# yatpor/bpc_baseline

Hardware: NVIDIA B200
Metric: matched+triangulated scenes/s with the ROI crops of every match (crops/s alongside) (higher is better)
Workload: dtype f64 geometry / u8+f32 crops

## Files before the change

### bpc_baseline_b200/_lib.py

```python
from __future__ import annotations

import ctypes as C
import os

HERE = os.path.dirname(os.path.abspath(__file__))
LIB_PATH = os.environ.get('BPC_LIB') or os.path.join(HERE, 'libbpc_b200.so')

_p = C.c_void_p
_i = C.c_int
_f = C.c_float
_sz = C.c_size_t

SIGNATURES = {
    'bpc_abi_version': (_i, []),
    'bpc_error_string': (C.c_char_p, [_i]),
    'bpc_launch_count': (C.c_ulonglong, []),
    'bpc_fundamental': (_i, [_p, _p, _i, _p, _p]),
    'bpc_cost_tensor': (_i, [_p, _p, _p, _i, _i, _p, _p]),
    'bpc_match_objects': (_i, [_p, _i, _i, _i, _i, _f, _p, _p, _p]),
    'bpc_match_workspace_bytes': (_sz, [_i, _i]),
    'bpc_match_triangulate': (_i, [_p, _p, _p, _p, _i, _i, _f, _i, C.c_double, _p, _p, _p, _p, _p, _p, _p, _sz, _p]),
    'bpc_pack_records_bytes': (_sz, [_i, _i]),
    'bpc_pack_records': (_i, [_p, _p, _p, _p, _p, _p, _i, _i, _i, _p, _p]),
    'bpc_triangulate': (_i, [_p, _p, _i, _p, _p]),
    'bpc_projection': (_i, [_p, _p, _i, _p, _p]),
    'bpc_reprojection_error': (_i, [_p, _p, _p, _i, _p, _p]),
    'bpc_epipolar_error': (_i, [_p, _p, _p, _i, _p, _p]),
    'bpc_epipolar_error_full': (_i, [_p, _p, _i, _p, _p]),
    'bpc_triangulate_views': (_i, [_p, _p, _i, _i, _p, _p]),
    'bpc_box_centers': (_i, [_p, _i, _p, _p]),
    'bpc_detections_from_yolo': (_i, [_p, _p, _p, _p, _i, _i, _f, _i, _p, _p, _p, _p]),
    'bpc_build_rois': (_i, [_p, _p, _p, _p, _i, _i, _i, _p, _p, _p]),
    'bpc_train_rois': (_i, [_p, _p, _p, _p, _i, _i, _i, _p, _p]),
    'bpc_roi_crop_workspace_bytes': (_sz, [_i, _i]),
    'bpc_roi_crop': (_i, [_p, _i, _i, _i, _p, _i, _p, _i, _i, _p, _i, _p, _p, _p, _p, _sz, _p]),
    'bpc_roi_crop_u8': (_i, [_p, _i, _i, _i, _p, _i, _p, _i, _i, _p, _p, _p, _p, _sz, _p]),
    'bpc_roi_crop_bf16': (_i, [_p, _i, _i, _i, _p, _i, _p, _i, _i, _p, _i, _p, _p, _p, _p, _sz, _p]),
    'bpc_normalise_lut': (_i, [_p, _p, _p, _p]),
    'bpc_crops_normalise': (_i, [_p, _p, _i, _i, _i, _p, _p, _p]),
    'bpc_color_jitter': (_i, [_p, _i, _i, _p, _p, _i, _p, _p, _p]),
}

_lib = None
ABI_VERSION = 2


class BpcError(RuntimeError):
    pass


def load():
    global _lib
    if _lib is not None:
        return _lib
    if not os.path.exists(LIB_PATH):
        raise BpcError(f'{LIB_PATH} not found: build it with `python -m bpc_baseline_b200.build` '
                       '(or __graft_entry__.build()); there is no CPU fallback')
    lib = C.CDLL(LIB_PATH)
    for name, (res, args) in SIGNATURES.items():
        fn = getattr(lib, name)
        fn.restype = res
        fn.argtypes = args
    if lib.bpc_abi_version() != ABI_VERSION:
        raise BpcError(f'ABI version mismatch: library {lib.bpc_abi_version()}, binding {ABI_VERSION}')
    _lib = lib
    return lib


def check(code: int, what: str):
    if code != 0:
        msg = load().bpc_error_string(code).decode()
        raise BpcError(f'{what} failed with code {code}: {msg}')


def launch_count() -> int:
    return int(load().bpc_launch_count())
```

### bpc_baseline_b200/batched.py

```python
from __future__ import annotations

import ctypes as C
from dataclasses import dataclass
from typing import Optional, Sequence

import numpy as np
import torch

from . import _lib

MEAN = (0.485, 0.456, 0.406)
STD = (0.229, 0.224, 0.225)


def _chk(t: torch.Tensor, dtype, name: str, ndim: Optional[int] = None):
    if not isinstance(t, torch.Tensor):
        raise TypeError(f'{name}: expected a torch.Tensor, got {type(t).__name__}')
    if not t.is_cuda:
        raise RuntimeError(f'{name}: must be a CUDA tensor (no CPU fallback)')
    if t.dtype != dtype:
        raise RuntimeError(f'{name}: dtype {t.dtype}, expected {dtype}')
    if not t.is_contiguous():
        raise RuntimeError(f'{name}: must be contiguous')
    if ndim is not None and t.dim() != ndim:
# ... 212 lines not shown
    e = torch.empty((n,), dtype=torch.float64, device=F.device)
    with torch.cuda.device(F.device):
        _lib.check(_lib.load().bpc_epipolar_error(_p(F), _p(pt1), _p(pt2), n, _p(e), _stream(F.device)), 'bpc_epipolar_error')
    return e


def epipolar_error_full(F: torch.Tensor, pts: torch.Tensor) -> torch.Tensor:
    _chk(F, torch.float64, 'F', 4); _chk(pts, torch.float64, 'pts', 3)
    n = F.shape[0]
    if tuple(F.shape) != (n, 3, 3, 3) or tuple(pts.shape) != (n, 3, 2):
        raise RuntimeError('expected F [n,3,3,3] and pts [n,3,2]')
    e = torch.empty((n,), dtype=torch.float64, device=F.device)
    with torch.cuda.device(F.device):
        _lib.check(_lib.load().bpc_epipolar_error_full(_p(F), _p(pts), n, _p(e), _stream(F.device)), 'bpc_epipolar_error_full')
    return e


def triangulate_views(P: torch.Tensor, pts: torch.Tensor) -> torch.Tensor:
    _chk(P, torch.float64, 'P', 4); _chk(pts, torch.float64, 'pts', 3)
    n, V = P.shape[0], P.shape[1]
    if tuple(P.shape) != (n, V, 3, 4) or tuple(pts.shape) != (n, V, 2) or not 2 <= V <= 8:
        raise RuntimeError('expected P [n,V,3,4] and pts [n,V,2] with 2 <= V <= 8')
    X = torch.empty((n, 3), dtype=torch.float64, device=P.device)
    with torch.cuda.device(P.device):
        _lib.check(_lib.load().bpc_triangulate_views(_p(P), _p(pts), n, V, _p(X), _stream(P.device)), 'bpc_triangulate_views')
    return X


def build_rois(boxes: torch.Tensor, idx: torch.Tensor, n: torch.Tensor, image_of_scene: torch.Tensor,
               rois: Optional[torch.Tensor] = None) -> tuple[torch.Tensor, torch.Tensor]:
    _chk(boxes, torch.int32, 'boxes', 4); _chk(idx, torch.int32, 'idx', 3); _chk(n, torch.int32, 'n', 1)
    _chk(image_of_scene, torch.int32, 'image_of_scene', 2)
    S, _, D, _ = boxes.shape
    K = idx.shape[1]
    dev = boxes.device
    if rois is None:
        rois = torch.empty((S * K * 3, 5), dtype=torch.int32, device=dev)
    else:
        _chk(rois, torch.int32, 'rois', 2)
        if rois.shape[0] < S * K * 3 or rois.shape[1] != 5:
            raise RuntimeError('rois must be int32 [>= S*Kmax*3, 5]')
    offs = torch.empty((S + 1,), dtype=torch.int32, device=dev)
    with torch.cuda.device(dev):
        _lib.check(_lib.load().bpc_build_rois(_p(boxes), _p(idx), _p(n), _p(image_of_scene), S, D, K, _p(offs), _p(rois),
                                              _stream(dev)), 'bpc_build_rois')
    return rois, offs


_LUT_CACHE: dict = {}


def normalise_lut(device, mean: Sequence[float] = MEAN, std: Sequence[float] = STD) -> torch.Tensor:
    device = torch.device(device)
    key = (device.index if device.index is not None else torch.cuda.current_device(), tuple(mean), tuple(std))
    if key not in _LUT_CACHE:
        lut = torch.empty((3, 256), dtype=torch.float32, device=device)
        m = (C.c_float * 3)(*[float(np.float32(v)) for v in mean])
        s = (C.c_float * 3)(*[float(np.float32(v)) for v in std])
        with torch.cuda.device(device):
            _lib.check(_lib.load().bpc_normalise_lut(m, s, _p(lut), _stream(device)), 'bpc_normalise_lut')
        _LUT_CACHE[key] = lut
    return _LUT_CACHE[key]


_WS_CACHE: dict = {}
MAX_ROIS_PER_LAUNCH = 32768
MAX_TARGET = 1024
MAX_ROI_WIDTH = 8192


def _crop_workspace(dev, R: int, T: int) -> torch.Tensor:
    need = int(_lib.load().bpc_roi_crop_workspace_bytes(int(R), int(T)))
    key = (dev.index if dev.index is not None else torch.cuda.current_device(), int(torch.cuda.current_stream(dev).cuda_stream))
    ws = _WS_CACHE.get(key)
    if ws is None or ws.numel() < need:
        ws = torch.empty((max(need, 1 << 16),), dtype=torch.uint8, device=dev)
        _WS_CACHE[key] = ws
    return ws


def _chk_status(status, R: int) -> None:
    if status is not None:
        _chk(status, torch.int32, 'status', 1)
        if status.shape[0] < R:
            raise RuntimeError('status must hold one int32 per ROI')


def _crop_args(images, rois, T, fill):
    _chk(images, torch.uint8, 'images', 4); _chk(rois, torch.int32, 'rois', 2)
    B, H, W, ch = images.shape
    if ch != 3 or rois.shape[1] != 5:
        raise RuntimeError('images must be [B,H,W,3] and rois [R,5]')
    if not 1 <= int(T) <= MAX_TARGET:
        raise RuntimeError(f'target size must be in 1..{MAX_TARGET}')
    f = (C.c_uint8 * 3)(*[int(v) for v in fill])
    return B, H, W, rois.shape[0], f


def roi_crop(images: torch.Tensor, rois: torch.Tensor, T: int = 256, fill=(255, 255, 255), swap_rb: bool = True,
             lut: Optional[torch.Tensor] = None, n_rois: Optional[torch.Tensor] = None, roi_first: int = 0,
             out: Optional[torch.Tensor] = None, status: Optional[torch.Tensor] = None) -> torch.Tensor:
    B, H, W, R, f = _crop_args(images, rois, T, fill)
    dev = images.device
    if lut is None:
        lut = normalise_lut(dev)
    _chk_lut(lut, dev)
    if out is None:
        out = torch.empty((R, 3, T, T), dtype=torch.float32, device=dev)
    else:
        _chk(out, torch.float32, 'out', 4)
        if out.shape[0] < R or tuple(out.shape[1:]) != (3, T, T):
            raise RuntimeError('out must be [>=R,3,T,T]')
        _chk_device(out, dev, 'out')
    _chk_status(status, R)
    if n_rois is not None:
        _chk(n_rois, torch.int32, 'n_rois')
    ws = _crop_workspace(dev, min(R, MAX_ROIS_PER_LAUNCH), T)
    with torch.cuda.device(dev):
        for lo in range(0, R, MAX_ROIS_PER_LAUNCH):
            r = min(MAX_ROIS_PER_LAUNCH, R - lo)
            _lib.check(_lib.load().bpc_roi_crop(_p(images), B, H, W, _p(rois[lo:lo + r]), r, _p(n_rois), int(roi_first) + lo, int(T),
                                                f, int(bool(swap_rb)), _p(lut), _p(out[lo:lo + r]),
                                                _p(status[lo:lo + r]) if status is not None else None,
                                                _p(ws), ws.numel(), _stream(dev)), 'bpc_roi_crop')
    return out


def roi_crop_bf16(images: torch.Tensor, rois: torch.Tensor, T: int = 256, fill=(255, 255, 255), swap_rb: bool = True,
                  lut: Optional[torch.Tensor] = None, n_rois: Optional[torch.Tensor] = None, roi_first: int = 0,
                  out: Optional[torch.Tensor] = None, status: Optional[torch.Tensor] = None) -> torch.Tensor:
    B, H, W, R, f = _crop_args(images, rois, T, fill)
    dev = images.device
    if lut is None:
        lut = normalise_lut(dev)
    _chk_lut(lut, dev)
    if out is None:
        out = torch.empty((R, 3, T, T), dtype=torch.bfloat16, device=dev, memory_format=torch.channels_last)
    else:
        if out.dtype != torch.bfloat16 or not out.is_cuda or out.dim() != 4 or out.shape[0] < R or tuple(out.shape[1:]) != (3, T, T) \
                or not out.is_contiguous(memory_format=torch.channels_last):
            raise RuntimeError('out must be a channels_last bfloat16 CUDA tensor [>=R,3,T,T]')
        _chk_device(out, dev, 'out')
    _chk_status(status, R)
    if n_rois is not None:
        _chk(n_rois, torch.int32, 'n_rois')
    ws = _crop_workspace(dev, min(R, MAX_ROIS_PER_LAUNCH), T)
    with torch.cuda.device(dev):
        for lo in range(0, R, MAX_ROIS_PER_LAUNCH):
            r = min(MAX_ROIS_PER_LAUNCH, R - lo)
            _lib.check(_lib.load().bpc_roi_crop_bf16(_p(images), B, H, W, _p(rois[lo:lo + r]), r, _p(n_rois), int(roi_first) + lo, int(T),
                                                     f, int(bool(swap_rb)), _p(lut), out[lo:lo + r].data_ptr(),
                                                     _p(status[lo:lo + r]) if status is not None else None,
                                                     _p(ws), ws.numel(), _stream(dev)), 'bpc_roi_crop_bf16')
    return out


def roi_crop_u8(images: torch.Tensor, rois: torch.Tensor, T: int = 256, fill=(255, 255, 255),
                   n_rois: Optional[torch.Tensor] = None, roi_first: int = 0, out: Optional[torch.Tensor] = None,
                status: Optional[torch.Tensor] = None) -> torch.Tensor:
    B, H, W, R, f = _crop_args(images, rois, T, fill)
    dev = images.device
    if out is None:
        out = torch.empty((R, T, T, 3), dtype=torch.uint8, device=dev)
    else:
        _chk(out, torch.uint8, 'out', 4)
        if out.shape[0] < R or tuple(out.shape[1:]) != (T, T, 3):
            raise RuntimeError('out must be uint8 [>=R,T,T,3]')
        _chk_device(out, dev, 'out')
    _chk_status(status, R)
    if n_rois is not None:
        _chk(n_rois, torch.int32, 'n_rois')
    ws = _crop_workspace(dev, min(R, MAX_ROIS_PER_LAUNCH), T)
    with torch.cuda.device(dev):
        for lo in range(0, R, MAX_ROIS_PER_LAUNCH):
            r = min(MAX_ROIS_PER_LAUNCH, R - lo)
            _lib.check(_lib.load().bpc_roi_crop_u8(_p(images), B, H, W, _p(rois[lo:lo + r]), r, _p(n_rois), int(roi_first) + lo, int(T),
                                                   f, _p(out[lo:lo + r]), _p(status[lo:lo + r]) if status is not None else None,
                                                   _p(ws), ws.numel(), _stream(dev)), 'bpc_roi_crop_u8')
    return out


def crops_normalise(sources: Sequence[torch.Tensor], T: int, swap_rb: bool = True, lut: Optional[torch.Tensor] = None,
                    out: Optional[torch.Tensor] = None, device=None) -> torch.Tensor:
    if not 1 <= len(sources) <= 16:
        raise RuntimeError('1..16 sources')
    for s in sources:
        _chk(s, torch.uint8, 'sources[*]', 4)
        if tuple(s.shape[1:]) != (T, T, 3):
            raise RuntimeError('every source must be uint8 [n,T,T,3]')
    dev = torch.device(device) if device is not None else sources[0].device
    if dev.type == 'cuda' and dev.index is None:
        dev = torch.device('cuda', torch.cuda.current_device())
    if lut is None:
        lut = normalise_lut(dev)
    _chk_lut(lut, dev)
    total = sum(int(s.shape[0]) for s in sources)
    if out is None:
        out = torch.empty((total, 3, T, T), dtype=torch.float32, device=dev)
    else:
        _chk(out, torch.float32, 'out', 4)
        if out.shape[0] < total or tuple(out.shape[1:]) != (3, T, T):
            raise RuntimeError('out must be [>=sum(n_s),3,T,T]')
        _chk_device(out, dev, 'out')
    ptrs = (C.c_void_p * len(sources))(*[s.data_ptr() if s.shape[0] else None for s in sources])
    counts = (C.c_int32 * len(sources))(*[int(s.shape[0]) for s in sources])
    with torch.cuda.device(dev):
        _lib.check(_lib.load().bpc_crops_normalise(ptrs, counts, len(sources), int(T), int(bool(swap_rb)), _p(lut), _p(out),
                                                   _stream(dev)), 'bpc_crops_normalise')
    return out


def color_jitter(canvases: torch.Tensor, order: torch.Tensor, factors: torch.Tensor, swap_rb: bool = False,
                 lut: Optional[torch.Tensor] = None, out: Optional[torch.Tensor] = None) -> torch.Tensor:
    _chk(canvases, torch.uint8, 'canvases', 4); _chk(order, torch.int32, 'order', 2); _chk(factors, torch.float32, 'factors', 2)
    n, T = canvases.shape[0], canvases.shape[1]
    if tuple(canvases.shape[1:]) != (T, T, 3) or tuple(order.shape) != (n, 4) or tuple(factors.shape) != (n, 4):
        raise RuntimeError('expected canvases [n,T,T,3], order [n,4] and factors [n,4]')
    if not 1 <= T <= MAX_TARGET:
        raise RuntimeError(f'target size must be in 1..{MAX_TARGET}')
    dev = canvases.device
    if order.device != dev or factors.device != dev:
        raise RuntimeError('canvases, order and factors must be on the same device')
    if lut is None:
        lut = normalise_lut(dev)
    _chk_lut(lut, dev)
    if out is None:
        out = torch.empty((n, 3, T, T), dtype=torch.float32, device=dev)
    else:
        _chk(out, torch.float32, 'out', 4)
        if out.shape[0] < n or tuple(out.shape[1:]) != (3, T, T):
            raise RuntimeError('out must be [>=n,3,T,T]')
        _chk_device(out, dev, 'out')
    with torch.cuda.device(dev):
        _lib.check(_lib.load().bpc_color_jitter(_p(canvases), n, T, _p(order), _p(factors), int(bool(swap_rb)), _p(lut), _p(out),
                                                _stream(dev)), 'bpc_color_jitter')
    return out


def train_rois(xywh: torch.Tensor, W: int, H: int, image: Optional[torch.Tensor] = None, scale: Optional[torch.Tensor] = None,
               shift: Optional[torch.Tensor] = None) -> torch.Tensor:
    _chk(xywh, torch.int32, 'xywh', 2)
    n = xywh.shape[0]
    if xywh.shape[1] != 4:
        raise RuntimeError('xywh must be [n,4]')
    if image is not None:
        _chk(image, torch.int32, 'image', 1)
    if scale is not None:
        _chk(scale, torch.float64, 'scale', 1)
    if shift is not None:
        _chk(shift, torch.int32, 'shift', 2)
        if scale is None:
            raise RuntimeError('shift needs scale (the reference draws both, data_utils.py:257-263)')
    for t, name in ((image, 'image'), (scale, 'scale'), (shift, 'shift')):
        if t is not None and t.shape[0] != n:
            raise RuntimeError(f'{name}: first dimension must be {n}')
    dev = xywh.device
    rois = torch.empty((n, 5), dtype=torch.int32, device=dev)
    with torch.cuda.device(dev):
        _lib.check(_lib.load().bpc_train_rois(_p(xywh), _p(image), _p(scale), _p(shift), n, int(W), int(H), _p(rois),
                                              _stream(dev)), 'bpc_train_rois')
    return rois
```

### bpc_baseline_b200/csrc/crop.cu

```cuda
#include <mutex>
#include <type_traits>

#include "crop_common.cuh"

namespace bpc {

#ifndef BPC_PREP_THREADS
#define BPC_PREP_THREADS 128
#endif
constexpr int PREP_THREADS = BPC_PREP_THREADS;

__device__ void src_row_records(float2* ysrc, int cap, const RoiGeom& g, int maxtaps, int tid, int* bad) {
    const int hpad = min(cap, ((g.h + STREAM_ROWS - 1) / STREAM_ROWS) * STREAM_ROWS + STREAM_ROWS);
    if (g.h + STREAM_ROWS > cap) *bad = 1;
    for (int s = tid; s < hpad; s += PREP_THREADS) ysrc[s] = make_float2(0.f, 0.f);
    __syncthreads();
    for (int d = tid; d < g.new_h && !*bad; d += PREP_THREADS) {
        int ys, yn, fl; float bf, bm, bl;
        area_taps(d, g.scale_y, g.h, ys, yn, bf, bm, bl, fl);
        const int prev_last = d > 0 ? area_last_tap(d - 1, g.scale_y, g.h) : -1;
        if (yn < 1 || yn > maxtaps || ys < prev_last || ys + yn > g.h) { *bad = 1; break; }
        for (int t = 0; t < yn; ++t) {
            const int s = ys + t;
            const bool shared_first = (t == 0 && s == prev_last);
// ... 704 lines not shown
                    }
                    const int b0 = __float_as_int(d.bf), b1 = __float_as_int(d.bm);
                    int o[3];
                    for (int c = 0; c < 3; ++c)
                        o[c] = ((((b0 * (HA[c] >> 4)) >> 16) + ((b1 * (HB[c] >> 4)) >> 16) + 2) >> 2) & 255;
                    out.px(roi, dy0 + yr, x, o[0], o[1], o[2]);
                } else if (incol) {
                    out.pad(roi, dy0 + yr, x);
                }
                ++yr;
            }
            if (yr < yb) chunk = yd[yr - ya].start;
        } else {
            while (yr < yb) {
                const YDesc d = yd[yr - ya];
                const int sy = d.start + t;
                if (sy >= chunk_end) break;
                if (active) {
                    const uint8_t* p = rowptr(sy) + 3 * xs;
                    if (regime == 1) {
                        if (cacheA != sy) {
                            float s0 = 0.f, s1 = 0.f, s2 = 0.f;
                            for (int k = 0; k < xn; ++k) {
                                const float a = (k == 0 && (xflags & 1)) ? af : ((k == xn - 1 && (xflags & 2)) ? al : am);
                                s0 = __fadd_rn(s0, __fmul_rn((float)p[3 * k + 0], a));
                                s1 = __fadd_rn(s1, __fmul_rn((float)p[3 * k + 1], a));
                                s2 = __fadd_rn(s2, __fmul_rn((float)p[3 * k + 2], a));
                            }
                            hA[0] = s0; hA[1] = s1; hA[2] = s2;
                            cacheA = sy;
                        }
                        const float beta = (t == 0 && (d.flags & 1)) ? d.bf : ((t == d.n - 1 && (d.flags & 2)) ? d.bl : d.bm);
                        for (int c = 0; c < 3; ++c) {
                            const float term = __fmul_rn(beta, hA[c]);
                            acc[c] = (t == 0) ? term : __fadd_rn(acc[c], term);
                        }
                    } else {
                        if (t == 0) { iacc[0] = 0; iacc[1] = 0; iacc[2] = 0; }
                        for (int k = 0; k < xn; ++k) {
                            iacc[0] += p[3 * k + 0]; iacc[1] += p[3 * k + 1]; iacc[2] += p[3 * k + 2];
                        }
                    }
                }
                ++t;
                if (t == d.n) {
                    if (active) {
                        int o[3];
                        if (regime == 1) {
                            for (int c = 0; c < 3; ++c) o[c] = min(255, max(0, __float2int_rn(acc[c])));
                        } else if (g.isx == 2 && g.isy == 2) {
                            for (int c = 0; c < 3; ++c) o[c] = (iacc[c] + 2) >> 2;
                        } else {
                            const float sc = __fdiv_rn(1.f, (float)(g.isx * g.isy));
                            for (int c = 0; c < 3; ++c) o[c] = min(255, max(0, __float2int_rn(__fmul_rn(__int2float_rn(iacc[c]), sc))));
                        }
                        out.px(roi, dy0 + yr, x, o[0], o[1], o[2]);
                    } else if (incol) {
                        out.pad(roi, dy0 + yr, x);
                    }
                    ++yr; t = 0;
                }
            }
            if (yr < yb) chunk = yd[yr - ya].start + t;
        }
    }
}

template <bool OUT_U8, int NTH, bool BF16 = false>
__global__ void __launch_bounds__(NTH)
bpc_crop_generic_kernel(const uint8_t* __restrict__ images, int B, int H, int W, const RoiGeom* __restrict__ geom,
                        const int32_t* __restrict__ glist, const int32_t* __restrict__ gcount, int T, int nbands,
                        uchar4 fill, int swap_rb, const float* __restrict__ lut_g, float* __restrict__ outf, uint8_t* __restrict__ outb) {
    extern __shared__ __align__(16) unsigned char raw[];
    __shared__ RoiGeom g;
    __shared__ YDesc yd[CROP_BAND];
    __shared__ float lut[OUT_U8 ? 1 : 3 * LUT_STRIDE];
    const int tid = threadIdx.x, nth = blockDim.x;
    const long long items = (long long)(*gcount) * nbands;
    if (blockIdx.x >= items) return;
    if (!OUT_U8)
        for (int e = tid; e < 768; e += nth) lut[(e >> 8) * LUT_STRIDE + (e & 255)] = lut_g[e];
    __syncthreads();
    Out<OUT_U8, BF16> out;
    out_init(out, outf, outb, lut, T, swap_rb, fill);
    for (long long item = blockIdx.x; item < items; item += gridDim.x) {
        const int roi = glist[item / nbands], band = (int)(item % nbands);
        __syncthreads();
        if (tid == 0) g = geom[roi];
        __syncthreads();
        crop_generic_band<OUT_U8, BF16>(raw, yd, out, g, roi, band, images, B, H, W, T, tid, nth);
    }
}

__global__ void bpc_lut_kernel(float m0, float m1, float m2, float s0, float s1, float s2, float* __restrict__ lut) {
    const int t = blockIdx.x * blockDim.x + threadIdx.x;
    if (t >= 768) return;
    const int c = t >> 8, v = t & 255;
    const float mean = c == 0 ? m0 : (c == 1 ? m1 : m2);
    const float sd = c == 0 ? s0 : (c == 1 ? s1 : s2);
    lut[t] = __fdiv_rn(__fsub_rn(__fdiv_rn((float)v, 255.f), mean), sd);
}

static int tensor_maps(const uint8_t* images, int B, int H, int W, bool aligned, TmapSet* out) {
    typedef CUresult (*EncodeFn)(CUtensorMap*, CUtensorMapDataType, cuuint32_t, void*, const cuuint64_t*, const cuuint64_t*,
                                 const cuuint32_t*, const cuuint32_t*, CUtensorMapInterleave, CUtensorMapSwizzle,
                                 CUtensorMapL2promotion, CUtensorMapFloatOOBfill);
    static std::mutex mu;
    static TmapSet cached;
    static const uint8_t* k_images = nullptr;
    static int k_B = 0, k_H = 0, k_W = 0, k_dev = -1;
    static EncodeFn encode = nullptr;
    std::lock_guard<std::mutex> lock(mu);
    if (!aligned) { memset(out, 0, sizeof(TmapSet)); return BPC_OK; }
    int dev = 0;
    cudaGetDevice(&dev);
    if (images == k_images && B == k_B && H == k_H && W == k_W && dev == k_dev) { *out = cached; return BPC_OK; }
    if (!encode) {
        cudaDriverEntryPointQueryResult q;
        void* fnp = nullptr;
        cudaError_t e = cudaGetDriverEntryPoint("cuTensorMapEncodeTiled", &fnp, cudaEnableDefault, &q);
        if (e != cudaSuccess) return (int)e;
        if (q != cudaDriverEntryPointSuccess || !fnp) return (int)cudaErrorNotSupported;
        encode = (EncodeFn)fnp;
    }
    const cuuint64_t gdim[2] = {(cuuint64_t)W * 3 / 4, (cuuint64_t)B * H};
    const cuuint64_t gstride[1] = {(cuuint64_t)W * 3};
    const cuuint32_t estr[2] = {1, 1};
    for (int i = 0; i < N_TMAPS; ++i) {
        const int pitch = i < 13 ? 64 + 32 * i : 512 + 64 * (i - 13);
        const cuuint32_t box[2] = {(cuuint32_t)pitch / 4, (cuuint32_t)tmap_rows(pitch)};
        const CUresult r = encode(&cached.m[i], CU_TENSOR_MAP_DATA_TYPE_UINT32, 2, (void*)images, gdim, gstride, box, estr,
                                  CU_TENSOR_MAP_INTERLEAVE_NONE, CU_TENSOR_MAP_SWIZZLE_NONE, BPC_L2_PROMO,
                                  CU_TENSOR_MAP_FLOAT_OOB_FILL_NONE);
        if (r != CUDA_SUCCESS) { k_images = nullptr; return (int)cudaErrorInvalidValue; }
    }
    for (int i = 0; i < N_TMAPS8; ++i) {
        const int pitch = 64 + 32 * i;
        const cuuint32_t box[2] = {(cuuint32_t)pitch / 4, (cuuint32_t)STREAM_ROWS};
        const CUresult r = encode(&cached.m8[i], CU_TENSOR_MAP_DATA_TYPE_UINT32, 2, (void*)images, gdim, gstride, box, estr,
                                  CU_TENSOR_MAP_INTERLEAVE_NONE, CU_TENSOR_MAP_SWIZZLE_NONE, BPC_L2_PROMO,
                                  CU_TENSOR_MAP_FLOAT_OOB_FILL_NONE);
        if (r != CUDA_SUCCESS) { k_images = nullptr; return (int)cudaErrorInvalidValue; }
    }
    k_images = images; k_B = B; k_H = H; k_W = W; k_dev = dev;
    *out = cached;
    return BPC_OK;
}

static size_t ws_off_xdesc(int R) { return (((size_t)R * sizeof(RoiGeom)) + 15) & ~(size_t)15; }
static size_t ws_off_ydesc(int R, int T) { return ws_off_xdesc(R) + (size_t)R * desc_stride(T) * sizeof(float4); }
static size_t ws_off_count(int R, int T) { return ws_off_ydesc(R, T) + (size_t)R * ydesc_stride(T) * sizeof(float4); }
static size_t crop_workspace_bytes(int R, int T) { return ws_off_count(R, T) + 64 + 2 * (size_t)R * sizeof(int32_t) + 64; }

template <bool OUT_U8, bool BF16 = false>
static int launch_crop(const uint8_t* images, int B, int H, int W, const int32_t* rois, int R, const int32_t* n_rois_dev,
                       int roi_first, int T, const uint8_t* fill, int swap_rb, const float* lut, float* outf, uint8_t* outb,
                       int32_t* status, void* workspace, size_t workspace_bytes, void* stream) {
    if (R < 0 || B < 1 || H < 1 || W < 1 || T < 1 || T > BPC_MAX_TARGET || !fill) return BPC_EINVAL;
    if (R > 0 && (!images || !rois || !workspace || (!OUT_U8 && (!lut || !outf)) || (OUT_U8 && !outb))) return BPC_EINVAL;
    if (((uintptr_t)images & 15) != 0 || ((uintptr_t)workspace & 15) != 0) return BPC_EALIGN;
    if (R == 0) return BPC_OK;
    if (workspace_bytes < crop_workspace_bytes(R, T)) return BPC_EWORKSPACE;
    const int nslot = (T + 31) / 32 + 1;
    if ((long long)R * nslot > 0x7fffffffLL) return BPC_ETOOBIG;
    cudaStream_t st = (cudaStream_t)stream;
    unsigned char* wsb = (unsigned char*)workspace;
    RoiGeom* geom = (RoiGeom*)wsb;
    float4* xdesc = (float4*)(wsb + ws_off_xdesc(R));
    float4* ydesc = (float4*)(wsb + ws_off_ydesc(R, T));
    int32_t* gcount = (int32_t*)(wsb + ws_off_count(R, T));
    int32_t* wcount = gcount + 4;
    int32_t* glist = gcount + 16;
    int32_t* list1 = glist + R;
    cudaError_t e = cudaMemsetAsync(gcount, 0, 64, st);
    if (e != cudaSuccess) return (int)e;
    const bool aligned = ((long long)W * 3) % 16 == 0 && (long long)W * 3 >= TMAP_MAX_PITCH;
    const bool use_cta = aligned && T <= CTA_MAX_T && (long long)W * 3 >= cta_pitch_max(T);
    if (BF16 && !use_cta) return BPC_EUNSUPPORTED;
    bpc_crop_prep_kernel<<<R, PREP_THREADS, 0, st>>>(images, B, H, W, rois, R, n_rois_dev, roi_first, T, (aligned ? 1 : 0) | (use_cta ? 2 : 0), geom, xdesc, ydesc,
                                            glist, gcount, status, use_cta ? list1 : nullptr);
    BPC_LAUNCH_CHECK();
    const uchar4 f4 = make_uchar4(fill[0], fill[1], fill[2], 0);
    if (use_cta) {
        const int rc = crop_cta_launch(OUT_U8 ? 1 : (BF16 ? 2 : 0), images, B, H, W, geom, xdesc, ydesc, list1, gcount, R, T, f4, swap_rb, lut,
                                       outf, outb, st);
        if (rc != BPC_OK) return rc;
    }
    if (!use_cta) {
        typedef void (*WarpFn)(const uint8_t*, int, int, int, const RoiGeom*, const float4*, const float4*, int32_t*, int, int, int,
                               uchar4, int, const float*, float*, uint8_t*, const TmapSet, const int32_t*);
        TmapSet tmaps;
        const int terr = tensor_maps(images, B, H, W, aligned, &tmaps);
        if (terr != BPC_OK) return terr;
        WarpFn fn;
        const bool sw = swap_rb != 0;
#define BPC_PICK(TTV)                                                                                                  \
    (aligned ? (sw ? bpc_crop_warp_kernel<OUT_U8, TTV, true, true> : bpc_crop_warp_kernel<OUT_U8, TTV, true, false>)   \
             : (sw ? bpc_crop_warp_kernel<OUT_U8, TTV, false, true> : bpc_crop_warp_kernel<OUT_U8, TTV, false, false>))
        if (OUT_U8) fn = aligned ? bpc_crop_warp_kernel<OUT_U8, 0, true, false> : bpc_crop_warp_kernel<OUT_U8, 0, false, false>;
        else if (T == 224) fn = BPC_PICK(224);
        else if (T == 256) fn = BPC_PICK(256);
        else fn = BPC_PICK(0);
#undef BPC_PICK
        e = cudaFuncSetAttribute(fn, cudaFuncAttributeMaxDynamicSharedMemorySize, WARPK_SMEM);
        if (e != cudaSuccess) return (int)e;
        const int cta_threads = 256;
        const long long nitems = (long long)R * nslot;
        const long long want = (nitems + WARPK_WARPS - 1) / WARPK_WARPS;
        int dev = 0, sms = 148, per_sm = 3;
        cudaGetDevice(&dev);
        cudaDeviceGetAttribute(&sms, cudaDevAttrMultiProcessorCount, dev);
        if (cudaOccupancyMaxActiveBlocksPerMultiprocessor(&per_sm, fn, cta_threads, WARPK_SMEM) != cudaSuccess || per_sm < 1) per_sm = 1;
        const long long slots = (long long)sms * per_sm;
        const int grid = (int)(want < slots ? want : slots);
        fn<<<grid, cta_threads, WARPK_SMEM, st>>>(images, B, H, W, geom, xdesc, ydesc, wcount, R, T, nslot, f4, swap_rb, lut, outf, outb, tmaps, use_cta ? list1 : nullptr);
        BPC_LAUNCH_CHECK();
    }
    const int nbands = (T + CROP_BAND - 1) / CROP_BAND;
    const long long max_items = (long long)R * nbands;
    const int grid = (int)(max_items < 148 * 2 ? max_items : 148 * 2);
    const int threads = ((T + 31) / 32) * 32;
    if (threads <= 256) {
        e = cudaFuncSetAttribute(bpc_crop_generic_kernel<OUT_U8, 256, BF16>, cudaFuncAttributeMaxDynamicSharedMemorySize, CROP_RAW_BYTES);
        if (e != cudaSuccess) return (int)e;
        bpc_crop_generic_kernel<OUT_U8, 256, BF16><<<grid, threads, CROP_RAW_BYTES, st>>>(images, B, H, W, geom, glist, gcount, T, nbands, f4,
                                                                                   swap_rb, lut, outf, outb);
    } else {
        e = cudaFuncSetAttribute(bpc_crop_generic_kernel<OUT_U8, 1024, BF16>, cudaFuncAttributeMaxDynamicSharedMemorySize, CROP_RAW_BYTES);
        if (e != cudaSuccess) return (int)e;
        bpc_crop_generic_kernel<OUT_U8, 1024, BF16><<<grid, threads, CROP_RAW_BYTES, st>>>(images, B, H, W, geom, glist, gcount, T, nbands, f4,
                                                                                    swap_rb, lut, outf, outb);
    }
    BPC_LAUNCH_CHECK();
    return BPC_OK;
}

}

using namespace bpc;

extern "C" size_t bpc_roi_crop_workspace_bytes(int R, int T) { return (R < 0 || T < 1 || T > BPC_MAX_TARGET) ? 0 : crop_workspace_bytes(R, T); }

extern "C" int bpc_roi_crop(const uint8_t* images, int B, int H, int W, const int32_t* rois, int R,
                            const int32_t* n_rois_dev, int roi_first, int T, const uint8_t* fill, int swap_rb,
                            const float* lut, float* out, int32_t* status, void* workspace, size_t workspace_bytes,
                            void* stream) {
    if (((uintptr_t)out & 15) != 0) return BPC_EALIGN;
    return launch_crop<false>(images, B, H, W, rois, R, n_rois_dev, roi_first, T, fill, swap_rb, lut, out, nullptr, status,
                              workspace, workspace_bytes, stream);
}

extern "C" int bpc_roi_crop_bf16(const uint8_t* images, int B, int H, int W, const int32_t* rois, int R,
                                 const int32_t* n_rois_dev, int roi_first, int T, const uint8_t* fill, int swap_rb,
                                 const float* lut, void* out, int32_t* status, void* workspace, size_t workspace_bytes,
                                 void* stream) {
    if (((uintptr_t)out & 15) != 0) return BPC_EALIGN;
    return launch_crop<false, true>(images, B, H, W, rois, R, n_rois_dev, roi_first, T, fill, swap_rb, lut, (float*)out, nullptr, status,
                                    workspace, workspace_bytes, stream);
}

extern "C" int bpc_roi_crop_u8(const uint8_t* images, int B, int H, int W, const int32_t* rois, int R,
                               const int32_t* n_rois_dev, int roi_first, int T, const uint8_t* fill, uint8_t* out,
                               int32_t* status, void* workspace, size_t workspace_bytes, void* stream) {
    return launch_crop<true>(images, B, H, W, rois, R, n_rois_dev, roi_first, T, fill, 0, nullptr, nullptr, out, status,
                             workspace, workspace_bytes, stream);
}

extern "C" int bpc_normalise_lut(const float* mean, const float* std_, float* lut, void* stream) {
    if (!mean || !std_ || !lut) return BPC_EINVAL;
    bpc_lut_kernel<<<3, 256, 0, (cudaStream_t)stream>>>(mean[0], mean[1], mean[2], std_[0], std_[1], std_[2], lut);
    BPC_LAUNCH_CHECK();
    return BPC_OK;
}
```

### bpc_baseline_b200/pipeline.py

```python
from __future__ import annotations

from typing import Callable, Optional

import numpy as np
import torch

from . import batched
from ._host import nvtx_range


class MatchCropPipeline:
    def __init__(self, S: int, Dmax: int, *, T: int = 224, chunk_rois: int = 16384, threshold=30,
                 swap_rb: bool = True, fill=(255, 255, 255), device='cuda', want_reproj: bool = True,
                 reproj_thresh: Optional[float] = None, crops: Optional[torch.Tensor] = None,
                 crop_dtype: torch.dtype = torch.float32):
        self.S, self.D, self.T = int(S), int(Dmax), int(T)
        self.device = torch.device(device)
        self.threshold = threshold
        self.swap_rb, self.fill, self.want_reproj, self.reproj_thresh = swap_rb, tuple(fill), want_reproj, reproj_thresh
        self.cap = self.S * self.D * 3
        self.chunk = max(1, min(int(chunk_rois), self.cap))
        dev = self.device
        self.rois = torch.zeros((self.cap, 5), dtype=torch.int32, device=dev)
        if crop_dtype not in (torch.float32, torch.bfloat16):
            raise RuntimeError('crop_dtype must be torch.float32 or torch.bfloat16')
        self.crop_dtype = crop_dtype
        if crop_dtype == torch.bfloat16:
            if crops is not None:
                raise RuntimeError('a caller-owned chunk buffer is float32 only')
            self.crops = torch.empty((self.chunk, 3, self.T, self.T), dtype=torch.bfloat16, device=dev, memory_format=torch.channels_last)
        elif crops is not None:
            if crops.dtype != torch.float32 or not crops.is_contiguous() or crops.numel() < self.chunk * 3 * self.T * self.T:
                raise RuntimeError('crops must be a contiguous float32 buffer of at least chunk_rois * 3 * T * T elements')
            self.crops = crops.view(-1)[:self.chunk * 3 * self.T * self.T].view(self.chunk, 3, self.T, self.T)
        else:
            self.crops = torch.empty((self.chunk, 3, self.T, self.T), dtype=torch.float32, device=dev)
        self.status = torch.zeros((self.cap,), dtype=torch.int32, device=dev)
        self.lut = batched.normalise_lut(dev)
        self._host = None
        self.last_crop_launches = 0

    def run_device(self, Ks, RTs, centers, counts, boxes, images, image_of_scene,
                   consumer: Optional[Callable[[torch.Tensor, int], None]] = None,
                   n_rois_host: Optional[int] = None, events=None):
        with nvtx_range('bpc.match'):
            res = batched.match_triangulate(Ks, RTs, centers, counts, self.threshold, want_reproj=self.want_reproj,
                                            reproj_thresh=self.reproj_thresh)
        with nvtx_range('bpc.build_rois'):
            rois, offs = batched.build_rois(boxes, res.idx, res.n, image_of_scene, rois=self.rois)
        total = offs[self.S:self.S + 1]
        if events is not None:
            events[0].record()
            events[1].record()
        upto = self.cap if n_rois_host is None else min(self.cap, int(n_rois_host))
        launches = 0
        for first in range(0, upto, self.chunk):
            r = min(self.chunk, self.cap - first)
            with nvtx_range('bpc.crop_chunk'):
                crop = batched.roi_crop_bf16 if self.crop_dtype == torch.bfloat16 else batched.roi_crop
                out = crop(images, rois[first:first + r], T=self.T, fill=self.fill, swap_rb=self.swap_rb,
                           lut=self.lut, n_rois=total, roi_first=first, out=self.crops, status=self.status[first:first + r])
            launches += 1
            if consumer is not None:
                consumer(out[:r], first)
        if events is not None:
            events[2].record()
        self.last_crop_launches = launches
        return res, offs

    def _alloc_host(self, images_shape):
        S, D, dev = self.S, self.D, self.device
        pin = lambda shape, dt: torch.empty(shape, dtype=dt).pin_memory()
        h = {
            'Ks': pin((S, 3, 3, 3), torch.float32), 'RTs': pin((S, 3, 4, 4), torch.float64),
            'boxes': pin((S, 3, D, 4), torch.int32), 'counts': pin((S, 3), torch.int32),
            'image_of_scene': pin((S, 3), torch.int32), 'images': pin(tuple(images_shape), torch.uint8),
            'idx': pin((S, D, 3), torch.int32), 'n': pin((S,), torch.int32), 'cost': pin((S, D), torch.float32),
            'X': pin((S, D, 3), torch.float64), 'n_rois': pin((1,), torch.int32),
        }
        d = {k: torch.empty(h[k].shape, dtype=h[k].dtype, device=dev)
             for k in ('Ks', 'RTs', 'boxes', 'counts', 'image_of_scene', 'images')}
        self._host = (h, d)

    def host_buffers(self, images_shape):
        if self._host is None or tuple(self._host[0]['images'].shape) != tuple(images_shape):
            self._alloc_host(images_shape)
        return self._host[0]

    def run_host(self, consumer=None, n_rois_host=None):
        h, d = self._host
        for k in d:
            d[k].copy_(h[k], non_blocking=True)
        centers = batched.box_centers(d['boxes'])
        res, offs = self.run_device(d['Ks'], d['RTs'], centers, d['counts'], d['boxes'], d['images'],
                                    d['image_of_scene'], consumer=consumer, n_rois_host=n_rois_host)
        h['idx'].copy_(res.idx, non_blocking=True)
        h['n'].copy_(res.n, non_blocking=True)
        h['cost'].copy_(res.cost, non_blocking=True)
        h['X'].copy_(res.X, non_blocking=True)
        h['n_rois'].copy_(offs[self.S:self.S + 1], non_blocking=True)
        torch.cuda.current_stream(self.device).synchronize()
        return h

    def run_host_stream(self, steps: int, refill: Optional[Callable[[dict, int], None]] = None,
                        on_result: Optional[Callable[[dict, int], None]] = None, consumer=None):
        h, d = self._host
        dev = self.device
        if not hasattr(self, '_stream_state'):
            d2 = {k: torch.empty_like(v) for k, v in d.items()}
            res_keys = ('idx', 'n', 'cost', 'X', 'n_rois')
            h2 = {k: torch.empty_like(h[k]).pin_memory() for k in res_keys}
            self._stream_state = {'d': (d, d2), 'hres': ({k: h[k] for k in res_keys}, h2),
                                  'copy': torch.cuda.Stream(device=dev)}
        st = self._stream_state
        main = torch.cuda.current_stream(dev)
        up_done = [torch.cuda.Event(), torch.cuda.Event()]
        free = [torch.cuda.Event(), torch.cuda.Event()]
        res_done = [torch.cuda.Event(), torch.cuda.Event()]
        host_read = [torch.cuda.Event(), torch.cuda.Event()]

        def upload(k):
            j = k & 1
            if refill is not None:
                if k >= 1:
                    host_read[(k - 1) & 1].synchronize()
                refill(h, k)
            with torch.cuda.stream(st['copy']):
                if k >= 2:
                    st['copy'].wait_event(free[j])
                for key, t in st['d'][j].items():
                    t.copy_(h[key], non_blocking=True)
                up_done[j].record(st['copy'])
                host_read[j].record(st['copy'])

        upload(0)
        for k in range(steps):
            j = k & 1
            if k + 1 < steps:
                upload(k + 1)
            main.wait_event(up_done[j])
            dj = st['d'][j]
            centers = batched.box_centers(dj['boxes'])
            res, offs = self.run_device(dj['Ks'], dj['RTs'], centers, dj['counts'], dj['boxes'], dj['images'],
                                        dj['image_of_scene'], consumer=consumer)
            free[j].record(main)
            if k >= 2:
                res_done[j].synchronize()
            hr = st['hres'][j]
            hr['idx'].copy_(res.idx, non_blocking=True)
            hr['n'].copy_(res.n, non_blocking=True)
            hr['cost'].copy_(res.cost, non_blocking=True)
            hr['X'].copy_(res.X, non_blocking=True)
            hr['n_rois'].copy_(offs[self.S:self.S + 1], non_blocking=True)
            res_done[j].record(main)
            if k >= 1:
                res_done[(k - 1) & 1].synchronize()
                if on_result is not None:
                    on_result(st['hres'][(k - 1) & 1], k - 1)
        res_done[(steps - 1) & 1].synchronize()
        if on_result is not None:
            on_result(st['hres'][(steps - 1) & 1], steps - 1)
        return st['hres'][(steps - 1) & 1]

    def h2d_bytes(self) -> int:
        h, d = self._host
        return int(sum(h[k].numel() * h[k].element_size() for k in d))

    def d2h_bytes(self) -> int:
        h, _ = self._host
        return int(sum(h[k].numel() * h[k].element_size() for k in ('idx', 'n', 'cost', 'X', 'n_rois')))


def algorithmic_crop_bytes(rois: np.ndarray, T: int, out_elem_bytes: int = 4) -> int:
    rois = np.asarray(rois, np.int64)
    w = rois[:, 3] - rois[:, 1]
    h = rois[:, 4] - rois[:, 2]
    return int((3 * w * h).sum() + len(rois) * (3 * T * T * out_elem_bytes + 20))
```

### include/bpc_b200.h

```cpp
#ifndef BPC_B200_H
#define BPC_B200_H

#include <stddef.h>
#include <stdint.h>

#ifdef __cplusplus
extern "C" {
#endif

#define BPC_ABI_VERSION 2

enum {
    BPC_OK = 0,
    BPC_EINVAL = -1,
    BPC_EALIGN = -2,
    BPC_EWORKSPACE = -3,
    BPC_ETOOBIG = -4,
    BPC_EUNSUPPORTED = -5
};

#define BPC_N_INFEASIBLE (-1)
#define BPC_N_OVERFLOW (-2)

#define BPC_MAX_DET 2048
#define BPC_MAX_ROI_WIDTH 8192
#define BPC_MAX_TARGET 1024

int bpc_abi_version(void);
const char* bpc_error_string(int code);

int bpc_fundamental(const float* Ks, const double* RTs, int S, double* F, void* stream);

int bpc_cost_tensor(const double* F, const double* centers, const int32_t* counts, int S, int Dmax,
                    float* cost, void* stream);

int bpc_match_objects(const float* cost, int S, int N, int M, int P, float threshold,
                      int32_t* idx, int32_t* n, void* stream);

size_t bpc_match_workspace_bytes(int S, int Dmax);
int bpc_match_triangulate(const float* Ks, const double* RTs, const double* centers, const int32_t* counts,
                          int S, int Dmax, float threshold, int has_reproj_thresh, double reproj_thresh,
                          int32_t* idx, int32_t* n, float* cost, double* X, double* reproj, double* F,
                          void* workspace, size_t workspace_bytes, void* stream);

size_t bpc_pack_records_bytes(int S, int Kmax);
int bpc_pack_records(const int32_t* idx, const int32_t* n, const float* cost, const double* X, const double* reproj,
                     const int32_t* scene_offset, int offset_div, int S, int Kmax, void* buf, void* stream);

int bpc_triangulate(const double* P, const double* pts, int n, double* X, void* stream);
int bpc_projection(const float* K, const double* RT, int n, double* P, void* stream);
int bpc_reprojection_error(const double* P, const double* X, const double* pts, int n, double* err, void* stream);

int bpc_epipolar_error(const double* F, const double* pt1, const double* pt2, int n, double* e, void* stream);
int bpc_epipolar_error_full(const double* F, const double* pts, int n, double* e, void* stream);
int bpc_triangulate_views(const double* P, const double* pts, int n, int V, double* X, void* stream);

int bpc_box_centers(const int32_t* boxes, int count, double* centers, void* stream);

int bpc_detections_from_yolo(const float* xyxy, const float* conf, const float* cls, const int32_t* nraw, int SC, int Nraw,
                             float conf_thresh, int Dmax, int32_t* boxes, double* centers, int32_t* counts, void* stream);

int bpc_build_rois(const int32_t* boxes, const int32_t* idx, const int32_t* n, const int32_t* image_of_scene,
                   int S, int Dmax, int Kmax, int32_t* scene_offset, int32_t* rois, void* stream);

int bpc_train_rois(const int32_t* xywh, const int32_t* image, const double* scale, const int32_t* shift, int n,
                   int W, int H, int32_t* rois, void* stream);

size_t bpc_roi_crop_workspace_bytes(int R, int T);
int bpc_roi_crop(const uint8_t* images, int B, int H, int W, const int32_t* rois, int R,
                 const int32_t* n_rois_dev, int roi_first, int T, const uint8_t* fill, int swap_rb,
                 const float* lut, float* out, int32_t* status,
                 void* workspace, size_t workspace_bytes, void* stream);
int bpc_roi_crop_u8(const uint8_t* images, int B, int H, int W, const int32_t* rois, int R,
                    const int32_t* n_rois_dev, int roi_first, int T, const uint8_t* fill,
                    uint8_t* out, int32_t* status,
                    void* workspace, size_t workspace_bytes, void* stream);
int bpc_roi_crop_bf16(const uint8_t* images, int B, int H, int W, const int32_t* rois, int R,
                      const int32_t* n_rois_dev, int roi_first, int T, const uint8_t* fill, int swap_rb,
                      const float* lut, void* out, int32_t* status,
                      void* workspace, size_t workspace_bytes, void* stream);
int bpc_normalise_lut(const float* mean_host3, const float* std_host3, float* lut, void* stream);

int bpc_crops_normalise(const uint8_t* const* srcs, const int32_t* counts, int n_src, int T, int swap_rb,
                        const float* lut, float* out, void* stream);

int bpc_color_jitter(const uint8_t* in, int n, int T, const int32_t* order, const float* factors, int swap_rb,
                     const float* lut, float* out, void* stream);

unsigned long long bpc_launch_count(void);

#ifdef __cplusplus
}
#endif
#endif
```

Measured before the change: 114,500.

## Split ROI crop into prepare/run and overlap prep on a side stream

Splits the crop launch into a prepare step (workspace memset plus per-ROI geometry/descriptor kernel) and a run step (the actual crop kernels). The pipeline then double-buffers two workspaces and issues the prepare for the next piece on a side stream while the current piece's crop runs on the main stream, synchronised with events. The goal is to hide the prep kernel's latency behind the crop work. In exchange it adds more Python-side launches, event records and waits per piece, plus a second workspace allocation.

```diff
diff --git a/bpc_baseline_b200/_lib.py b/bpc_baseline_b200/_lib.py
--- a/bpc_baseline_b200/_lib.py
+++ b/bpc_baseline_b200/_lib.py
@@ -36,6 +36,9 @@
     'bpc_roi_crop': (_i, [_p, _i, _i, _i, _p, _i, _p, _i, _i, _p, _i, _p, _p, _p, _p, _sz, _p]),
     'bpc_roi_crop_u8': (_i, [_p, _i, _i, _i, _p, _i, _p, _i, _i, _p, _p, _p, _p, _sz, _p]),
     'bpc_roi_crop_bf16': (_i, [_p, _i, _i, _i, _p, _i, _p, _i, _i, _p, _i, _p, _p, _p, _p, _sz, _p]),
+    'bpc_roi_crop_prepare': (_i, [_p, _i, _i, _i, _p, _i, _p, _i, _i, _p, _p, _sz, _p]),
+    'bpc_roi_crop_run': (_i, [_p, _i, _i, _i, _i, _i, _p, _i, _p, _p, _p, _sz, _p]),
+    'bpc_roi_crop_bf16_run': (_i, [_p, _i, _i, _i, _i, _i, _p, _i, _p, _p, _p, _sz, _p]),
     'bpc_normalise_lut': (_i, [_p, _p, _p, _p]),
     'bpc_crops_normalise': (_i, [_p, _p, _i, _i, _i, _p, _p, _p]),
     'bpc_color_jitter': (_i, [_p, _i, _i, _p, _p, _i, _p, _p, _p]),
diff --git a/bpc_baseline_b200/batched.py b/bpc_baseline_b200/batched.py
--- a/bpc_baseline_b200/batched.py
+++ b/bpc_baseline_b200/batched.py
@@ -388,6 +388,63 @@
                                                      f, int(bool(swap_rb)), _p(lut), out[lo:lo + r].data_ptr(),
                                                      _p(status[lo:lo + r]) if status is not None else None,
                                                      _p(ws), ws.numel(), _stream(dev)), 'bpc_roi_crop_bf16')
+    return out
+
+
+def crop_workspace_bytes(R: int, T: int) -> int:
+    return int(_lib.load().bpc_roi_crop_workspace_bytes(int(R), int(T)))
+
+
+def _chk_workspace(ws: torch.Tensor, R: int, T: int, dev) -> None:
+    _chk(ws, torch.uint8, 'workspace', 1)
+    _chk_device(ws, dev, 'workspace')
+    if not 0 <= R <= MAX_ROIS_PER_LAUNCH:
+        raise RuntimeError(f'at most {MAX_ROIS_PER_LAUNCH} ROIs per prepare / run')
+    if ws.numel() < crop_workspace_bytes(R, T):
+        raise RuntimeError('workspace must hold crop_workspace_bytes(R, T) bytes')
+
+
+def roi_crop_prepare(images: torch.Tensor, rois: torch.Tensor, T: int, workspace: torch.Tensor,
+                     n_rois: Optional[torch.Tensor] = None, roi_first: int = 0, status: Optional[torch.Tensor] = None) -> None:
+    B, H, W, R, _ = _crop_args(images, rois, T, (0, 0, 0))
+    dev = images.device
+    _chk_workspace(workspace, R, T, dev)
+    _chk_status(status, R)
+    if n_rois is not None:
+        _chk(n_rois, torch.int32, 'n_rois')
+    with torch.cuda.device(dev):
+        _lib.check(_lib.load().bpc_roi_crop_prepare(_p(images), B, H, W, _p(rois), R, _p(n_rois), int(roi_first), int(T),
+                                                    _p(status), _p(workspace), workspace.numel(), _stream(dev)),
+                   'bpc_roi_crop_prepare')
+
+
+def roi_crop_run(images: torch.Tensor, R: int, T: int, workspace: torch.Tensor, out: torch.Tensor, fill=(255, 255, 255),
+                 swap_rb: bool = True, lut: Optional[torch.Tensor] = None) -> torch.Tensor:
+    _chk(images, torch.uint8, 'images', 4)
+    B, H, W, ch = images.shape
+    if ch != 3 or not 1 <= int(T) <= MAX_TARGET:
+        raise RuntimeError(f'images must be [B,H,W,3] and the target size in 1..{MAX_TARGET}')
+    f = (C.c_uint8 * 3)(*[int(v) for v in fill])
+    dev = images.device
+    R = int(R)
+    _chk_workspace(workspace, R, T, dev)
+    if lut is None:
+        lut = normalise_lut(dev)
+    _chk_lut(lut, dev)
+    if out.dtype == torch.bfloat16:
+        if not out.is_cuda or out.dim() != 4 or out.shape[0] < R or tuple(out.shape[1:]) != (3, T, T) \
+                or not out.is_contiguous(memory_format=torch.channels_last):
+            raise RuntimeError('out must be a channels_last bfloat16 CUDA tensor [>=R,3,T,T]')
+        fn, name = _lib.load().bpc_roi_crop_bf16_run, 'bpc_roi_crop_bf16_run'
+    else:
+        _chk(out, torch.float32, 'out', 4)
+        if out.shape[0] < R or tuple(out.shape[1:]) != (3, T, T):
+            raise RuntimeError('out must be [>=R,3,T,T]')
+        fn, name = _lib.load().bpc_roi_crop_run, 'bpc_roi_crop_run'
+    _chk_device(out, dev, 'out')
+    with torch.cuda.device(dev):
+        _lib.check(fn(_p(images), B, H, W, R, int(T), f, int(bool(swap_rb)), _p(lut), out.data_ptr(), _p(workspace),
+                      workspace.numel(), _stream(dev)), name)
     return out
 
 
diff --git a/bpc_baseline_b200/csrc/crop.cu b/bpc_baseline_b200/csrc/crop.cu
--- a/bpc_baseline_b200/csrc/crop.cu
+++ b/bpc_baseline_b200/csrc/crop.cu
@@ -880,34 +880,69 @@
 static size_t ws_off_count(int R, int T) { return ws_off_ydesc(R, T) + (size_t)R * ydesc_stride(T) * sizeof(float4); }
 static size_t crop_workspace_bytes(int R, int T) { return ws_off_count(R, T) + 64 + 2 * (size_t)R * sizeof(int32_t) + 64; }
 
-template <bool OUT_U8, bool BF16 = false>
-static int launch_crop(const uint8_t* images, int B, int H, int W, const int32_t* rois, int R, const int32_t* n_rois_dev,
-                       int roi_first, int T, const uint8_t* fill, int swap_rb, const float* lut, float* outf, uint8_t* outb,
-                       int32_t* status, void* workspace, size_t workspace_bytes, void* stream) {
-    if (R < 0 || B < 1 || H < 1 || W < 1 || T < 1 || T > BPC_MAX_TARGET || !fill) return BPC_EINVAL;
-    if (R > 0 && (!images || !rois || !workspace || (!OUT_U8 && (!lut || !outf)) || (OUT_U8 && !outb))) return BPC_EINVAL;
+struct CropWs {
+    RoiGeom* geom; float4* xdesc; float4* ydesc;
+    int32_t* gcount;
+    int32_t* glist; int32_t* list1;
+};
+static CropWs crop_ws(void* workspace, int R, int T) {
+    unsigned char* wsb = (unsigned char*)workspace;
+    CropWs w;
+    w.geom = (RoiGeom*)wsb;
+    w.xdesc = (float4*)(wsb + ws_off_xdesc(R));
+    w.ydesc = (float4*)(wsb + ws_off_ydesc(R, T));
+    w.gcount = (int32_t*)(wsb + ws_off_count(R, T));
+    w.glist = w.gcount + 16;
+    w.list1 = w.glist + R;
+    return w;
+}
+static bool pool_aligned(int W) { return ((long long)W * 3) % 16 == 0 && (long long)W * 3 >= TMAP_MAX_PITCH; }
+static bool pool_use_cta(int W, int T) { return pool_aligned(W) && T <= CTA_MAX_T && (long long)W * 3 >= cta_pitch_max(T); }
+
+static int crop_check(const uint8_t* images, int B, int H, int W, int R, int T, const void* workspace, size_t workspace_bytes) {
+    if (R < 0 || B < 1 || H < 1 || W < 1 || T < 1 || T > BPC_MAX_TARGET) return BPC_EINVAL;
+    if (R > 0 && (!images || !workspace)) return BPC_EINVAL;
     if (((uintptr_t)images & 15) != 0 || ((uintptr_t)workspace & 15) != 0) return BPC_EALIGN;
     if (R == 0) return BPC_OK;
     if (workspace_bytes < crop_workspace_bytes(R, T)) return BPC_EWORKSPACE;
+    if ((long long)R * ((T + 31) / 32 + 1) > 0x7fffffffLL) return BPC_ETOOBIG;
+    return BPC_OK;
+}
+
+static int crop_prepare(const uint8_t* images, int B, int H, int W, const int32_t* rois, int R, const int32_t* n_rois_dev,
+                        int roi_first, int T, int32_t* status, void* workspace, size_t workspace_bytes, cudaStream_t st) {
+    if (R > 0 && !rois) return BPC_EINVAL;
+    const int chk = crop_check(images, B, H, W, R, T, workspace, workspace_bytes);
+    if (chk != BPC_OK || R == 0) return chk;
+    const CropWs ws = crop_ws(workspace, R, T);
+    cudaError_t e = cudaMemsetAsync(ws.gcount, 0, 64, st);
+    if (e != cudaSuccess) return (int)e;
+    const bool aligned = pool_aligned(W), use_cta = pool_use_cta(W, T);
+    bpc_crop_prep_kernel<<<R, PREP_THREADS, 0, st>>>(images, B, H, W, rois, R, n_rois_dev, roi_first, T,
+                                            (aligned ? 1 : 0) | (use_cta ? 2 : 0), ws.geom, ws.xdesc, ws.ydesc, ws.glist, ws.gcount,
+                                            status, use_cta ? ws.list1 : nullptr);
+    BPC_LAUNCH_CHECK();
+    return BPC_OK;
+}
+
+template <bool OUT_U8, bool BF16 = false>
+static int crop_run(const uint8_t* images, int B, int H, int W, int R, int T, const uint8_t* fill, int swap_rb, const float* lut,
+                    float* outf, uint8_t* outb, void* workspace, size_t workspace_bytes, cudaStream_t st) {
+    if (!fill || (R > 0 && ((!OUT_U8 && (!lut || !outf)) || (OUT_U8 && !outb)))) return BPC_EINVAL;
+    const int chk = crop_check(images, B, H, W, R, T, workspace, workspace_bytes);
+    if (chk != BPC_OK || R == 0) return chk;
+    const bool aligned = pool_aligned(W), use_cta = pool_use_cta(W, T);
+    if (BF16 && !use_cta) return BPC_EUNSUPPORTED;
+    const CropWs ws = crop_ws(workspace, R, T);
+    RoiGeom* geom = ws.geom;
+    float4* xdesc = ws.xdesc;
+    float4* ydesc = ws.ydesc;
+    int32_t* gcount = ws.gcount;
+    int32_t* wcount = gcount + 4;
+    int32_t* glist = ws.glist;
+    int32_t* list1 = ws.list1;
     const int nslot = (T + 31) / 32 + 1;
-    if ((long long)R * nslot > 0x7fffffffLL) return BPC_ETOOBIG;
-    cudaStream_t st = (cudaStream_t)stream;
-    unsigned char* wsb = (unsigned char*)workspace;
-    RoiGeom* geom = (RoiGeom*)wsb;
-    float4* xdesc = (float4*)(wsb + ws_off_xdesc(R));
-    float4* ydesc = (float4*)(wsb + ws_off_ydesc(R, T));
-    int32_t* gcount = (int32_t*)(wsb + ws_off_count(R, T));
-    int32_t* wcount = gcount + 4;
-    int32_t* glist = gcount + 16;
-    int32_t* list1 = glist + R;
-    cudaError_t e = cudaMemsetAsync(gcount, 0, 64, st);
-    if (e != cudaSuccess) return (int)e;
-    const bool aligned = ((long long)W * 3) % 16 == 0 && (long long)W * 3 >= TMAP_MAX_PITCH;
-    const bool use_cta = aligned && T <= CTA_MAX_T && (long long)W * 3 >= cta_pitch_max(T);
-    if (BF16 && !use_cta) return BPC_EUNSUPPORTED;
-    bpc_crop_prep_kernel<<<R, PREP_THREADS, 0, st>>>(images, B, H, W, rois, R, n_rois_dev, roi_first, T, (aligned ? 1 : 0) | (use_cta ? 2 : 0), geom, xdesc, ydesc,
-                                            glist, gcount, status, use_cta ? list1 : nullptr);
-    BPC_LAUNCH_CHECK();
+    cudaError_t e;
     const uchar4 f4 = make_uchar4(fill[0], fill[1], fill[2], 0);
     if (use_cta) {
         const int rc = crop_cta_launch(OUT_U8 ? 1 : (BF16 ? 2 : 0), images, B, H, W, geom, xdesc, ydesc, list1, gcount, R, T, f4, swap_rb, lut,
@@ -963,6 +998,23 @@
     return BPC_OK;
 }
 
+template <bool OUT_U8, bool BF16 = false>
+static int launch_crop(const uint8_t* images, int B, int H, int W, const int32_t* rois, int R, const int32_t* n_rois_dev,
+                       int roi_first, int T, const uint8_t* fill, int swap_rb, const float* lut, float* outf, uint8_t* outb,
+                       int32_t* status, void* workspace, size_t workspace_bytes, void* stream) {
+    if (R < 0 || B < 1 || H < 1 || W < 1 || T < 1 || T > BPC_MAX_TARGET || !fill) return BPC_EINVAL;
+    if (R > 0 && (!images || !rois || !workspace || (!OUT_U8 && (!lut || !outf)) || (OUT_U8 && !outb))) return BPC_EINVAL;
+    if (((uintptr_t)images & 15) != 0 || ((uintptr_t)workspace & 15) != 0) return BPC_EALIGN;
+    if (R == 0) return BPC_OK;
+    if (workspace_bytes < crop_workspace_bytes(R, T)) return BPC_EWORKSPACE;
+    if ((long long)R * ((T + 31) / 32 + 1) > 0x7fffffffLL) return BPC_ETOOBIG;
+    if (BF16 && !pool_use_cta(W, T)) return BPC_EUNSUPPORTED;
+    cudaStream_t st = (cudaStream_t)stream;
+    const int rc = crop_prepare(images, B, H, W, rois, R, n_rois_dev, roi_first, T, status, workspace, workspace_bytes, st);
+    if (rc != BPC_OK) return rc;
+    return crop_run<OUT_U8, BF16>(images, B, H, W, R, T, fill, swap_rb, lut, outf, outb, workspace, workspace_bytes, st);
+}
+
 }
 
 using namespace bpc;
@@ -987,6 +1039,25 @@
                                     workspace, workspace_bytes, stream);
 }
 
+extern "C" int bpc_roi_crop_prepare(const uint8_t* images, int B, int H, int W, const int32_t* rois, int R,
+                                    const int32_t* n_rois_dev, int roi_first, int T, int32_t* status, void* workspace,
+                                    size_t workspace_bytes, void* stream) {
+    return crop_prepare(images, B, H, W, rois, R, n_rois_dev, roi_first, T, status, workspace, workspace_bytes, (cudaStream_t)stream);
+}
+
+extern "C" int bpc_roi_crop_run(const uint8_t* images, int B, int H, int W, int R, int T, const uint8_t* fill, int swap_rb,
+                                const float* lut, float* out, void* workspace, size_t workspace_bytes, void* stream) {
+    if (((uintptr_t)out & 15) != 0) return BPC_EALIGN;
+    return crop_run<false>(images, B, H, W, R, T, fill, swap_rb, lut, out, nullptr, workspace, workspace_bytes, (cudaStream_t)stream);
+}
+
+extern "C" int bpc_roi_crop_bf16_run(const uint8_t* images, int B, int H, int W, int R, int T, const uint8_t* fill, int swap_rb,
+                                     const float* lut, void* out, void* workspace, size_t workspace_bytes, void* stream) {
+    if (((uintptr_t)out & 15) != 0) return BPC_EALIGN;
+    return crop_run<false, true>(images, B, H, W, R, T, fill, swap_rb, lut, (float*)out, nullptr, workspace, workspace_bytes,
+                                 (cudaStream_t)stream);
+}
+
 extern "C" int bpc_roi_crop_u8(const uint8_t* images, int B, int H, int W, const int32_t* rois, int R,
                                const int32_t* n_rois_dev, int roi_first, int T, const uint8_t* fill, uint8_t* out,
                                int32_t* status, void* workspace, size_t workspace_bytes, void* stream) {
diff --git a/bpc_baseline_b200/pipeline.py b/bpc_baseline_b200/pipeline.py
--- a/bpc_baseline_b200/pipeline.py
+++ b/bpc_baseline_b200/pipeline.py
@@ -37,6 +37,9 @@
             self.crops = torch.empty((self.chunk, 3, self.T, self.T), dtype=torch.float32, device=dev)
         self.status = torch.zeros((self.cap,), dtype=torch.int32, device=dev)
         self.lut = batched.normalise_lut(dev)
+        piece = min(self.chunk, batched.MAX_ROIS_PER_LAUNCH)
+        self._ws = [torch.empty((batched.crop_workspace_bytes(piece, self.T),), dtype=torch.uint8, device=dev) for _ in range(2)]
+        self._side = torch.cuda.Stream(device=dev, priority=0)
         self._host = None
         self.last_crop_launches = 0
 
@@ -54,15 +57,40 @@
             events[1].record()
         upto = self.cap if n_rois_host is None else min(self.cap, int(n_rois_host))
         launches = 0
-        for first in range(0, upto, self.chunk):
-            r = min(self.chunk, self.cap - first)
-            with nvtx_range('bpc.crop_chunk'):
-                crop = batched.roi_crop_bf16 if self.crop_dtype == torch.bfloat16 else batched.roi_crop
-                out = crop(images, rois[first:first + r], T=self.T, fill=self.fill, swap_rb=self.swap_rb,
-                           lut=self.lut, n_rois=total, roi_first=first, out=self.crops, status=self.status[first:first + r])
-            launches += 1
-            if consumer is not None:
-                consumer(out[:r], first)
+        pieces = [(first, lo, min(batched.MAX_ROIS_PER_LAUNCH, first + min(self.chunk, self.cap - first) - lo))
+                  for first in range(0, upto, self.chunk)
+                  for lo in range(first, first + min(self.chunk, self.cap - first), batched.MAX_ROIS_PER_LAUNCH)]
+        if pieces:
+            main, side = torch.cuda.current_stream(self.device), self._side
+            prepared = [torch.cuda.Event(), torch.cuda.Event()]
+            cropped = [torch.cuda.Event(), torch.cuda.Event()]
+            rois_ready = torch.cuda.Event()
+            rois_ready.record(main)
+
+            def prepare(i):
+                _, lo, n = pieces[i]
+                j = i & 1
+                with torch.cuda.stream(side):
+                    side.wait_event(cropped[j] if i >= 2 else rois_ready)
+                    batched.roi_crop_prepare(images, rois[lo:lo + n], self.T, self._ws[j], n_rois=total, roi_first=lo,
+                                             status=self.status[lo:lo + n])
+                    prepared[j].record(side)
+
+            prepare(0)
+            for i, (first, lo, n) in enumerate(pieces):
+                j = i & 1
+                with nvtx_range('bpc.crop_chunk'):
+                    main.wait_event(prepared[j])
+                    batched.roi_crop_run(images, n, self.T, self._ws[j], self.crops[lo - first:lo - first + n], fill=self.fill,
+                                         swap_rb=self.swap_rb, lut=self.lut)
+                    cropped[j].record(main)
+                    if i + 1 < len(pieces):
+                        prepare(i + 1)
+                if i + 1 == len(pieces) or pieces[i + 1][0] != first:
+                    r = min(self.chunk, self.cap - first)
+                    launches += 1
+                    if consumer is not None:
+                        consumer(self.crops[:r], first)
         if events is not None:
             events[2].record()
         self.last_crop_launches = launches
diff --git a/include/bpc_b200.h b/include/bpc_b200.h
--- a/include/bpc_b200.h
+++ b/include/bpc_b200.h
@@ -79,6 +79,13 @@
                       const int32_t* n_rois_dev, int roi_first, int T, const uint8_t* fill, int swap_rb,
                       const float* lut, void* out, int32_t* status,
                       void* workspace, size_t workspace_bytes, void* stream);
+int bpc_roi_crop_prepare(const uint8_t* images, int B, int H, int W, const int32_t* rois, int R,
+                         const int32_t* n_rois_dev, int roi_first, int T, int32_t* status,
+                         void* workspace, size_t workspace_bytes, void* stream);
+int bpc_roi_crop_run(const uint8_t* images, int B, int H, int W, int R, int T, const uint8_t* fill, int swap_rb,
+                     const float* lut, float* out, void* workspace, size_t workspace_bytes, void* stream);
+int bpc_roi_crop_bf16_run(const uint8_t* images, int B, int H, int W, int R, int T, const uint8_t* fill, int swap_rb,
+                          const float* lut, void* out, void* workspace, size_t workspace_bytes, void* stream);
 int bpc_normalise_lut(const float* mean_host3, const float* std_host3, float* lut, void* stream);
 
 int bpc_crops_normalise(const uint8_t* const* srcs, const int32_t* counts, int n_src, int T, int swap_rb,
```

Measured after the change: 116,300 (median of 6 runs). +1.6%, better.
